# arcee-ai/DALM

Hardware: NVIDIA H100
Metric: RAG-e2e train-step samples/sec (bge-large + Llama-2-7B, bs=18) (higher is better)
Workload: dtype bf16

## Files before the change

### dalm_b200/csrc/gemm_wgmma.cu

```cuda
#include "common.cuh"
#include "ptx.cuh"
#include <cudaTypedefs.h>
#include <mutex>
#include <unordered_map>

namespace dalm {
using namespace ptx;

enum class Epi {
  Plain,
  SwiGLU,
  RoPE,
  GeluPair,
  NormRoPE,
};

struct GemmEpilogue {
  void* out;
  long long ldo;
  int out_f32;
  const float* bias;
  const void* resid;
  long long ldr;
  int resid_f32;
  int act;
  float alpha;
  int M, N, K;
  DropCfg drop;
  int group_m;
  const float* rope_cos; const float* rope_sin;
  int rope_L, rope_cols;
  const float* q_norm; const float* k_norm;
  int nq_heads;
  float norm_eps;
  float* norm_rstd; long long ld_rstd;
  int norm_pre;
  int l2_hints;
};

__device__ __forceinline__ void tile_coords(int tile, int num_m, int num_n, int gm, int& m_blk, int& n_blk) {
  if (gm <= 0) { m_blk = tile % num_m; n_blk = tile / num_m; return; }
  const int band_tiles = gm * num_n;
  const int band = tile / band_tiles;
  const int r = tile - band * band_tiles;
  const int m0 = band * gm;
  const int h = min(gm, num_m - m0);
  const int n = r / h;
  m_blk = m0 + (r - n * h);
  n_blk = (band & 1) ? (num_n - 1 - n) : n;
}

template <bool PRE = false>
__device__ __forceinline__ void epilogue_math(const GemmEpilogue& ep, const uint32_t* v, float* f, int row, int col0, bool row_ok,
                                              const float4* rpre = nullptr) {
  const int N = ep.N;
#pragma unroll
  for (int i = 0; i < 32; ++i) f[i] = __uint_as_float(v[i]) * ep.alpha;
  if (ep.bias) {
#pragma unroll
    for (int i = 0; i < 32; ++i) if (col0 + i < N) f[i] += __ldg(ep.bias + col0 + i);
  }
  if (ep.act == 1) {
#pragma unroll
    for (int i = 0; i < 32; ++i) f[i] = gelu_erf(f[i]);
  }
  if (ep.drop.p > 0.f) {
    const unsigned long long dstream = drop_stream(ep.drop);
    const unsigned long long base = ((unsigned long long)row * (unsigned long long)N + (unsigned long long)col0) >> 3;
#pragma unroll
    for (int g = 0; g < 4; ++g) {
      float sc[8];
      drop_scale8(ep.drop, dstream, base + g, sc);
#pragma unroll
      for (int j = 0; j < 8; ++j) f[g * 8 + j] *= sc[j];
    }
  }
  if constexpr (PRE) {
#pragma unroll
    for (int g = 0; g < 8; ++g) { f[g * 4 + 0] += rpre[g].x; f[g * 4 + 1] += rpre[g].y; f[g * 4 + 2] += rpre[g].z; f[g * 4 + 3] += rpre[g].w; }
  } else if (ep.resid && row_ok) {
    if (ep.resid_f32) {
      const float* r = reinterpret_cast<const float*>(ep.resid) + (size_t)row * ep.ldr + col0;
#pragma unroll
      for (int g = 0; g < 8; ++g) {
        if (col0 + g * 4 < N) {
          const float4 t = *reinterpret_cast<const float4*>(r + g * 4);
          f[g * 4 + 0] += t.x; f[g * 4 + 1] += t.y; f[g * 4 + 2] += t.z; f[g * 4 + 3] += t.w;
        }
      }
    } else {
      const __nv_bfloat16* r = reinterpret_cast<const __nv_bfloat16*>(ep.resid) + (size_t)row * ep.ldr + col0;
#pragma unroll
      for (int g = 0; g < 4; ++g) {
        if (col0 + g * 8 < N) {
          const bf16x8 t = *reinterpret_cast<const bf16x8*>(r + g * 8);
          float tf[8];
          unpack8(t, tf);
          if (ep.act == 2) {
#pragma unroll
            for (int i = 0; i < 8; ++i) f[g * 8 + i] = __bfloat162float(__float2bfloat16_rn(f[g * 8 + i])) * gelu_erf_grad(tf[i]);
          } else {
#pragma unroll
            for (int i = 0; i < 8; ++i) f[g * 8 + i] += tf[i];
          }
        }
      }
    }
  }
}

__device__ __forceinline__ void acc_ld32(const float* p, uint32_t* v) {
#pragma unroll
  for (int g = 0; g < 8; ++g) {
    const float4 t = *reinterpret_cast<const float4*>(p + g * 4);
    v[g * 4 + 0] = __float_as_uint(t.x); v[g * 4 + 1] = __float_as_uint(t.y);
    v[g * 4 + 2] = __float_as_uint(t.z); v[g * 4 + 3] = __float_as_uint(t.w);
  }
}

constexpr int kStageTileBytes = 128 * 128;
constexpr int kEpiGroups = 2;
constexpr int kGemmThreads = 128 + kEpiGroups * 128;
template <int BN, Epi EPI>
__device__ __forceinline__ void epilogue_drain_tile(const GemmEpilogue& ep, const CUtensorMap* tmap_out, const CUtensorMap* tmap_out2,
                                                    unsigned char* staging, int grp, const float* arow, int row_in_tile, int tile_row0,
                                                    int tile_col0) {
  static_assert(BN == 256 || EPI == Epi::Plain || EPI == Epi::GeluPair, "the SwiGLU and RoPE epilogues need 256-wide tiles");
  const int N = ep.N;
  const int row = tile_row0 + row_in_tile;
  const bool row_ok = row < ep.M;
  constexpr bool F32_OUT = EPI == Epi::Plain;
  const int sb_cols = (F32_OUT && ep.out_f32) ? 32 : 64;
  const bool issuer = (threadIdx.x == 128 + grp * 128);
  unsigned char* tile = staging + grp * kStageTileBytes;
  unsigned char* st = tile + row_in_tile * 128;
  const int sw = row_in_tile & 7;
  const bool rpf = F32_OUT && ep.out_f32 && ep.resid != nullptr && ep.resid_f32;
  float4 rnext[8];
  auto fetch_resid = [&](int cc) {
    const int cg0 = tile_col0 + cc;
    const float* r = reinterpret_cast<const float*>(ep.resid) + (size_t)row * ep.ldr + cg0;
#pragma unroll
    for (int g = 0; g < 8; ++g)
      rnext[g] = (row_ok && cc < BN && cg0 + g * 4 < N) ? *reinterpret_cast<const float4*>(r + g * 4) : make_float4(0.f, 0.f, 0.f, 0.f);
  };
  if (rpf) fetch_resid(grp * sb_cols);
#pragma unroll 1
  for (int c = grp * sb_cols; c < BN; c += kEpiGroups * sb_cols) {
    const int col0 = tile_col0 + c;
    if (col0 >= N) break;
    if (issuer) bulk_wait_read<0>();
    named_bar_sync(1 + grp, 128);
    if (F32_OUT && ep.out_f32) {
      uint32_t v[32]; float f[32];
      acc_ld32(arow + c, v);
      if (rpf) {
        epilogue_math<true>(ep, v, f, row, col0, row_ok, rnext);
        fetch_resid(c + kEpiGroups * sb_cols);
      } else {
        epilogue_math<false>(ep, v, f, row, col0, row_ok);
      }
#pragma unroll
      for (int g = 0; g < 8; ++g)
        *reinterpret_cast<float4*>(st + ((g ^ sw) << 4)) = make_float4(f[g * 4], f[g * 4 + 1], f[g * 4 + 2], f[g * 4 + 3]);
    } else if (EPI == Epi::RoPE && col0 < ep.rope_cols) {
      const bool second = ((col0 >> 6) & 1) != 0;
      const int cp = second ? c - 64 : c + 64;
      const int colp = tile_col0 + cp;
      const int pos = row_ok ? (row % ep.rope_L) : 0;
      const float* cs = ep.rope_cos + (size_t)pos * 64;
      const float* sn = ep.rope_sin + (size_t)pos * 64;
#pragma unroll
      for (int h = 0; h < 2; ++h) {
        uint32_t vo[32], vq[32]; float f[32];
        acc_ld32(arow + (c + h * 32), vo);
        acc_ld32(arow + (cp + h * 32), vq);
        float cc[32], ss[32];
#pragma unroll
        for (int i = 0; i < 32; i += 4) {
          *reinterpret_cast<float4*>(cc + i) = __ldg(reinterpret_cast<const float4*>(cs + h * 32 + i));
          *reinterpret_cast<float4*>(ss + i) = __ldg(reinterpret_cast<const float4*>(sn + h * 32 + i));
        }
#pragma unroll
        for (int i = 0; i < 32; ++i) {
          float own = __uint_as_float(vo[i]), oth = __uint_as_float(vq[i]);
          if (ep.bias) {
            own += __ldg(ep.bias + col0 + h * 32 + i);
            oth += __ldg(ep.bias + colp + h * 32 + i);
          }
          f[i] = second ? fmaf(own, cc[i], oth * ss[i]) : fmaf(own, cc[i], -oth * ss[i]);
        }
#pragma unroll
        for (int g = 0; g < 4; ++g)
          *reinterpret_cast<bf16x8*>(st + (((h * 4 + g) ^ sw) << 4)) = pack8(f + g * 8);
      }
    } else if (EPI == Epi::NormRoPE && col0 < ep.rope_cols) {
      const bool second = ((col0 >> 6) & 1) != 0;
      const int cp = second ? c - 64 : c + 64;
      const int colp = tile_col0 + cp;
      const int c1 = second ? cp : c;
      const int head = col0 >> 7;
      const float* nw = head < ep.nq_heads ? ep.q_norm : ep.k_norm;
      const int jo = second ? 64 : 0, jp = 64 - jo;
      float ss = 0.f;
#pragma unroll 1
      for (int h = 0; h < 4; ++h) {
        uint32_t v[32];
        acc_ld32(arow + (c1 + h * 32), v);
#pragma unroll
        for (int i = 0; i < 32; ++i) {
          float x = __uint_as_float(v[i]);
          if (ep.bias) x += __ldg(ep.bias + tile_col0 + c1 + h * 32 + i);
          ss = fmaf(x, x, ss);
        }
      }
      const float rstd = rsqrtf(ss * (1.f / 128.f) + ep.norm_eps);
      if (ep.norm_rstd && row_ok && !second) ep.norm_rstd[(size_t)row * ep.ld_rstd + head] = rstd;
      const int pos = row_ok ? (row % ep.rope_L) : 0;
      const float* cs = ep.rope_cos + (size_t)pos * 64;
      const float* sn = ep.rope_sin + (size_t)pos * 64;
#pragma unroll
      for (int h = 0; h < 2; ++h) {
        uint32_t vo[32], vq[32]; float f[32];
        acc_ld32(arow + (c + h * 32), vo);
        acc_ld32(arow + (cp + h * 32), vq);
        float cc[32], ss2[32];
#pragma unroll
        for (int i = 0; i < 32; i += 4) {
          *reinterpret_cast<float4*>(cc + i) = __ldg(reinterpret_cast<const float4*>(cs + h * 32 + i));
          *reinterpret_cast<float4*>(ss2 + i) = __ldg(reinterpret_cast<const float4*>(sn + h * 32 + i));
        }
#pragma unroll
        for (int i = 0; i < 32; ++i) {
          float own = __uint_as_float(vo[i]), oth = __uint_as_float(vq[i]);
          if (ep.bias) {
            own += __ldg(ep.bias + col0 + h * 32 + i);
            oth += __ldg(ep.bias + colp + h * 32 + i);
          }
          own = own * rstd * __ldg(nw + jo + h * 32 + i);
          oth = oth * rstd * __ldg(nw + jp + h * 32 + i);
          f[i] = second ? fmaf(own, cc[i], oth * ss2[i]) : fmaf(own, cc[i], -oth * ss2[i]);
        }
#pragma unroll
        for (int g = 0; g < 4; ++g)
          *reinterpret_cast<bf16x8*>(st + (((h * 4 + g) ^ sw) << 4)) = pack8(f + g * 8);
      }
      fence_proxy_async();
      named_bar_sync(1 + grp, 128);
      if (issuer) {
        if (ep.l2_hints & 4) tma_store_2d_hint(tmap_out, tile, col0, tile_row0, l2_policy_evict_first());
        else                 tma_store_2d(tmap_out, tile, col0, tile_row0);
        bulk_commit();
      }
      if (!ep.norm_pre) continue;
      if (issuer) bulk_wait_read<0>();
      named_bar_sync(1 + grp, 128);
#pragma unroll
      for (int h = 0; h < 2; ++h) {
        uint32_t v[32]; float f[32];
        acc_ld32(arow + (c + h * 32), v);
#pragma unroll
        for (int i = 0; i < 32; ++i) {
          f[i] = __uint_as_float(v[i]);
          if (ep.bias) f[i] += __ldg(ep.bias + col0 + h * 32 + i);
        }
#pragma unroll
        for (int g = 0; g < 4; ++g)
          *reinterpret_cast<bf16x8*>(st + (((h * 4 + g) ^ sw) << 4)) = pack8(f + g * 8);
      }
      fence_proxy_async();
      named_bar_sync(1 + grp, 128);
      if (issuer) {
        tma_store_2d(tmap_out2, tile, col0, tile_row0);
        bulk_commit();
      }
      continue;
    } else if (EPI == Epi::GeluPair) {
      bf16x8 pk[8];
#pragma unroll
      for (int h = 0; h < 2; ++h) {
        if (col0 + h * 32 < N) {
          uint32_t v[32]; float f[32];
          acc_ld32(arow + (c + h * 32), v);
          epilogue_math(ep, v, f, row, col0 + h * 32, row_ok);
#pragma unroll
          for (int g = 0; g < 4; ++g) pk[h * 4 + g] = pack8(f + g * 8);
        } else {
#pragma unroll
          for (int g = 0; g < 4; ++g) pk[h * 4 + g] = bf16x8{};
        }
      }
#pragma unroll
      for (int g = 0; g < 8; ++g) *reinterpret_cast<bf16x8*>(st + ((g ^ sw) << 4)) = pk[g];
      fence_proxy_async();
      named_bar_sync(1 + grp, 128);
      if (issuer) {
        if (ep.l2_hints & 4) tma_store_2d_hint(tmap_out, tile, col0, tile_row0, l2_policy_evict_first());
        else                 tma_store_2d(tmap_out, tile, col0, tile_row0);
        bulk_commit();
      }
#pragma unroll
      for (int g = 0; g < 8; ++g) {
        float x[8];
        unpack8(pk[g], x);
#pragma unroll
        for (int i = 0; i < 8; ++i) x[i] = gelu_erf(x[i]);
        pk[g] = pack8(x);
      }
      if (issuer) bulk_wait_read<0>();
      named_bar_sync(1 + grp, 128);
#pragma unroll
      for (int g = 0; g < 8; ++g) *reinterpret_cast<bf16x8*>(st + ((g ^ sw) << 4)) = pk[g];
      fence_proxy_async();
      named_bar_sync(1 + grp, 128);
      if (issuer) {
        tma_store_2d(tmap_out2, tile, col0, tile_row0);
        bulk_commit();
      }
      continue;
    } else {
#pragma unroll
      for (int h = 0; h < 2; ++h) {
        if (col0 + h * 32 < N) {
          uint32_t v[32]; float f[32];
          acc_ld32(arow + (c + h * 32), v);
          epilogue_math(ep, v, f, row, col0 + h * 32, row_ok);
#pragma unroll
          for (int g = 0; g < 4; ++g)
            *reinterpret_cast<bf16x8*>(st + (((h * 4 + g) ^ sw) << 4)) = pack8(f + g * 8);
        }
      }
    }
    fence_proxy_async();
    named_bar_sync(1 + grp, 128);
    if (issuer) {
      if (ep.l2_hints & 4) tma_store_2d_hint(tmap_out, tile, col0, tile_row0, l2_policy_evict_first());
      else                 tma_store_2d(tmap_out, tile, col0, tile_row0);
      bulk_commit();
    }
  }
  if constexpr (EPI == Epi::SwiGLU) {
    const int j = grp;
    const int acol0 = (tile_col0 >> 1) + j * 64;
    if (issuer) bulk_wait_read<0>();
    named_bar_sync(1 + grp, 128);
#pragma unroll
    for (int h = 0; h < 2; ++h) {
      uint32_t vg[32], vu[32]; float f[32];
      acc_ld32(arow + (j * 64 + h * 32), vg);
      acc_ld32(arow + (128 + j * 64 + h * 32), vu);
#pragma unroll
      for (int i = 0; i < 32; ++i) {
        const float g = __uint_as_float(vg[i]);
        f[i] = g / (1.f + __expf(-g)) * __uint_as_float(vu[i]);
      }
#pragma unroll
      for (int g4 = 0; g4 < 4; ++g4) *reinterpret_cast<bf16x8*>(st + (((h * 4 + g4) ^ sw) << 4)) = pack8(f + g4 * 8);
    }
    fence_proxy_async();
    named_bar_sync(1 + grp, 128);
    if (issuer) {
      if (ep.l2_hints & 4) tma_store_2d_hint(tmap_out2, tile, acol0, tile_row0, l2_policy_evict_first());
      else                 tma_store_2d(tmap_out2, tile, acol0, tile_row0);
      bulk_commit();
    }
  }
}

template <int BN> struct GemmCfg {
  static constexpr int BM = 128, BK = 64;
  static constexpr int A_BYTES = BM * BK * 2;
  static constexpr int B_BYTES = BN * BK * 2;
  static constexpr int STAGE_BYTES = A_BYTES + B_BYTES;
  static constexpr int STAGES = (BN == 256) ? 4 : (BN == 128 ? 6 : 8);
  static constexpr int ACC_LD = BN + 4;
  static constexpr int SMEM_BYTES = STAGES * STAGE_BYTES + 2 * kStageTileBytes + 1024  + 256 ;
  static_assert(BM * ACC_LD * 4 <= STAGES * STAGE_BYTES, "the accumulator tile reuses the stage ring");
  static_assert(SMEM_BYTES <= 232448, "exceeds 227 KB of shared memory per block");
};

template <int BN, int TA, int TB>
__device__ __forceinline__ void wgmma_tile(float* d, uint64_t da, uint64_t db, int scale_d) {
  if constexpr (BN == 256) wgmma_m64n256k16<TA, TB>(d, da, db, scale_d);
  else if constexpr (BN == 128) wgmma_m64n128k16<TA, TB>(d, da, db, scale_d);
  else wgmma_m64n64k16<TA, TB>(d, da, db, scale_d);
}

template <int BN, int LAYOUT, Epi EPI, int CL>
__global__ void __launch_bounds__(kGemmThreads, 1)
gemm_bf16_tn_kernel(const __grid_constant__ CUtensorMap tmap_a, const __grid_constant__ CUtensorMap tmap_b,
                    const __grid_constant__ CUtensorMap tmap_out, const __grid_constant__ CUtensorMap tmap_out2, const GemmEpilogue ep) {
  using Cfg = GemmCfg<BN>;
  constexpr int BM = Cfg::BM, BK = Cfg::BK, STAGES = Cfg::STAGES;
  static_assert(CL == 1 || (LAYOUT == 0 && EPI == Epi::Plain), "the cluster kernel takes the plain TN layout");
  extern __shared__ unsigned char smem_raw[];
  unsigned char* smem = reinterpret_cast<unsigned char*>((reinterpret_cast<uintptr_t>(smem_raw) + 1023) & ~uintptr_t(1023));
  unsigned char* staging = smem + STAGES * Cfg::STAGE_BYTES;
  uint64_t* full_bar  = reinterpret_cast<uint64_t*>(staging + 2 * kStageTileBytes);
  uint64_t* empty_bar = full_bar + STAGES;
  uint64_t* epi_bar   = empty_bar + STAGES;
  float* acc_smem = reinterpret_cast<float*>(smem);

  const int warp = threadIdx.x >> 5, lane = threadIdx.x & 31;
  const uint32_t rank = CL == 2 ? cluster_ctarank() : 0u;
  const int M = ep.M, N = ep.N, K = ep.K;
  const int num_m = (M + CL * BM - 1) / (CL * BM), num_n = (N + BN - 1) / BN;
  const int num_tiles = num_m * num_n;
  const int num_kb = (K + BK - 1) / BK;
  const int unit = blockIdx.x / CL, num_units = gridDim.x / CL;
  const int group_m = CL == 2 ? 0 : ep.group_m;

  if (threadIdx.x == 0) {
    prefetch_tmap(&tmap_a);
    prefetch_tmap(&tmap_b);
    prefetch_tmap(&tmap_out);
    if constexpr (EPI == Epi::SwiGLU || EPI == Epi::GeluPair || EPI == Epi::NormRoPE) prefetch_tmap(&tmap_out2);
  }
  if (threadIdx.x == 32) {
    for (int s = 0; s < STAGES; ++s) { mbar_init(&full_bar[s], 1); mbar_init(&empty_bar[s], 8 * CL); }
    mbar_init(epi_bar, 8 * CL);
    fence_mbar_init();
  }
  if constexpr (CL == 2) cluster_sync_all();
  else __syncthreads();

  if (warp < 4) {
    asm volatile("setmaxnreg.dec.sync.aligned.u32 40;" ::: "memory");
    if (warp == 0 && lane == 0) {
      int stage = 0; uint32_t phase = 0;
      const bool hint_a = (ep.l2_hints & 1) != 0, hint_b = (ep.l2_hints & 2) != 0;
      const uint64_t pol_a = hint_a ? l2_policy_evict_last() : 0ull, pol_b = hint_b ? l2_policy_evict_first() : 0ull;
      auto load = [](void* dst, const CUtensorMap* tm, uint64_t* bar, int c0, int c1, bool hinted, uint64_t pol) {
        if (hinted) tma_load_2d_hint(dst, tm, bar, c0, c1, pol);
        else        tma_load_2d(dst, tm, bar, c0, c1);
      };
      int it = 0;
      for (int tile = unit; tile < num_tiles; tile += num_units, ++it) {
        int m_blk, n_blk;
        tile_coords(tile, num_m, num_n, group_m, m_blk, n_blk);
        if (it > 0) mbar_wait(epi_bar, (uint32_t)(it - 1) & 1u);
        for (int kb = 0; kb < num_kb; ++kb) {
          mbar_wait(&empty_bar[stage], phase ^ 1);
          unsigned char* sa = smem + stage * Cfg::STAGE_BYTES;
          unsigned char* sb = sa + Cfg::A_BYTES;
          mbar_arrive_expect_tx(&full_bar[stage], Cfg::STAGE_BYTES);
          if constexpr (CL == 2) {
            load(sa, &tmap_a, &full_bar[stage], kb * BK, (m_blk * CL + (int)rank) * BM, hint_a, pol_a);
            tma_load_2d_multicast(sb + rank * (Cfg::B_BYTES / 2), &tmap_b, &full_bar[stage], kb * BK, n_blk * BN + (int)rank * (BN / 2), 0x3);
          } else {
            if constexpr (LAYOUT == 2) {
#pragma unroll
              for (int c = 0; c < BM / 64; ++c) load(sa + c * 8192, &tmap_a, &full_bar[stage], m_blk * BM + c * 64, kb * BK, hint_a, pol_a);
            } else {
              load(sa, &tmap_a, &full_bar[stage], kb * BK, m_blk * BM, hint_a, pol_a);
            }
            if constexpr (LAYOUT >= 1) {
#pragma unroll
              for (int c = 0; c < BN / 64; ++c) load(sb + c * 8192, &tmap_b, &full_bar[stage], n_blk * BN + c * 64, kb * BK, hint_b, pol_b);
            } else {
              load(sb, &tmap_b, &full_bar[stage], kb * BK, n_blk * BN, hint_b, pol_b);
            }
          }
          if (++stage == STAGES) { stage = 0; phase ^= 1; }
        }
      }
    }
  } else {
    asm volatile("setmaxnreg.inc.sync.aligned.u32 232;" ::: "memory");
    const int grp = (warp - 4) >> 2;
    const int q = warp & 3;
    constexpr int TA = LAYOUT == 2 ? 1 : 0, TB = LAYOUT >= 1 ? 1 : 0;
    constexpr uint64_t a_step = TA ? 128 : 2, b_step = TB ? 128 : 2;
    const uint32_t a_off = (uint32_t)grp * 8192u;
    int stage = 0; uint32_t phase = 0;
    for (int tile = unit; tile < num_tiles; tile += num_units) {
      int m_blk, n_blk;
      tile_coords(tile, num_m, num_n, group_m, m_blk, n_blk);
      float acc[BN / 2];
      int prev = -1;
      for (int kb = 0; kb < num_kb; ++kb) {
        mbar_wait(&full_bar[stage], phase);
        const uint32_t sa = smem_u32(smem + stage * Cfg::STAGE_BYTES);
        const uint32_t sb = sa + Cfg::A_BYTES;
        const uint64_t adesc = TA ? make_sw128_mnmajor_desc(sa + a_off, 8192, 1024) : make_sw128_kmajor_desc(sa + a_off);
        const uint64_t bdesc = TB ? make_sw128_mnmajor_desc(sb, 8192, 1024) : make_sw128_kmajor_desc(sb);
        wgmma_fence();
#pragma unroll
        for (int k = 0; k < BK / 16; ++k)
          wgmma_tile<BN, TA, TB>(acc, adesc + a_step * (uint64_t)k, bdesc + b_step * (uint64_t)k, (kb | k) != 0 ? 1 : 0);
        wgmma_commit();
        wgmma_wait<1>();
        if (prev >= 0 && lane == 0) {
          mbar_arrive(&empty_bar[prev]);
          if constexpr (CL == 2) mbar_arrive_remote(&empty_bar[prev], rank ^ 1u);
        }
        prev = stage;
        if (++stage == STAGES) { stage = 0; phase ^= 1; }
      }
      wgmma_wait<0>();
      if (lane == 0) {
        mbar_arrive(&empty_bar[prev]);
        if constexpr (CL == 2) mbar_arrive_remote(&empty_bar[prev], rank ^ 1u);
      }
      named_bar_sync(3, 256);
      {
        const int r0 = grp * 64 + q * 16 + (lane >> 2);
        float* p0 = acc_smem + (size_t)r0 * Cfg::ACC_LD + 2 * (lane & 3);
        float* p1 = p0 + 8 * Cfg::ACC_LD;
#pragma unroll
        for (int j = 0; j < BN / 8; ++j) {
          *reinterpret_cast<float2*>(p0 + 8 * j) = make_float2(acc[4 * j], acc[4 * j + 1]);
          *reinterpret_cast<float2*>(p1 + 8 * j) = make_float2(acc[4 * j + 2], acc[4 * j + 3]);
        }
      }
      named_bar_sync(3, 256);
      const int row_in_tile = q * 32 + lane;
      epilogue_drain_tile<BN, EPI>(ep, &tmap_out, &tmap_out2, staging, grp, acc_smem + (size_t)row_in_tile * Cfg::ACC_LD,
                                   row_in_tile, (m_blk * CL + (int)rank) * BM, n_blk * BN);
      fence_proxy_async();
      __syncwarp();
      if (lane == 0) {
        mbar_arrive(epi_bar);
        if constexpr (CL == 2) mbar_arrive_remote(epi_bar, rank ^ 1u);
      }
    }
    if ((threadIdx.x & 127) == 0) bulk_wait<0>();
  }
  if constexpr (CL == 2) cluster_sync_all();
}

static PFN_cuTensorMapEncodeTiled_v12000 get_encode_fn() {
  static PFN_cuTensorMapEncodeTiled_v12000 fn = nullptr;
  static std::once_flag once;
  std::call_once(once, [] {
    void* p = nullptr;
    cudaDriverEntryPointQueryResult qres;
    if (cudaGetDriverEntryPoint("cuTensorMapEncodeTiled", &p, cudaEnableDefault, &qres) == cudaSuccess &&
        qres == cudaDriverEntryPointSuccess)
      fn = reinterpret_cast<PFN_cuTensorMapEncodeTiled_v12000>(p);
  });
  return fn;
}

struct TmapKey {
  const void* ptr; long long rows, cols, ld; int box_rows; int f32;
  bool operator==(const TmapKey& o) const {
    return ptr == o.ptr && rows == o.rows && cols == o.cols && ld == o.ld && box_rows == o.box_rows && f32 == o.f32;
  }
};
struct TmapKeyHash {
  size_t operator()(const TmapKey& k) const {
    size_t h = reinterpret_cast<size_t>(k.ptr);
    h = h * 1000003u ^ (size_t)k.rows; h = h * 1000003u ^ (size_t)k.cols;
    h = h * 1000003u ^ (size_t)k.ld;   h = h * 1000003u ^ (size_t)(k.box_rows * 2 + k.f32);
    return h;
  }
};
static std::unordered_map<TmapKey, CUtensorMap, TmapKeyHash> g_tmaps;
static std::mutex g_tmap_mu;

int get_tmap(const void* ptr, long long rows, long long cols, long long ld, int box_rows, CUtensorMap* out, int f32) {
  TmapKey key{ptr, rows, cols, ld, box_rows, f32};
  {
    std::lock_guard<std::mutex> g(g_tmap_mu);
    auto it = g_tmaps.find(key);
    if (it != g_tmaps.end()) { *out = it->second; return 0; }
  }
  auto fn = get_encode_fn();
  DALM_REQUIRE(fn != nullptr, "gemm: cuTensorMapEncodeTiled driver entry point unavailable");
  DALM_REQUIRE((reinterpret_cast<uintptr_t>(ptr) & 15) == 0, "gemm: operand base %p is not 16-byte aligned", ptr);
  DALM_REQUIRE((ld % (f32 ? 4 : 8)) == 0, "gemm: row stride %lld is not a multiple of 16 bytes", ld);
  cuuint64_t dims[2] = {(cuuint64_t)cols, (cuuint64_t)rows};
  cuuint64_t strides[1] = {(cuuint64_t)ld * (f32 ? 4 : 2)};
  cuuint32_t box[2] = {f32 ? 32u : 64u, (cuuint32_t)box_rows};
  cuuint32_t estr[2] = {1u, 1u};
  CUtensorMap m;
  CUresult r = fn(&m, f32 ? CU_TENSOR_MAP_DATA_TYPE_FLOAT32 : CU_TENSOR_MAP_DATA_TYPE_BFLOAT16, 2, const_cast<void*>(ptr), dims, strides, box, estr,
                  CU_TENSOR_MAP_INTERLEAVE_NONE, CU_TENSOR_MAP_SWIZZLE_128B, CU_TENSOR_MAP_L2_PROMOTION_L2_256B,
                  CU_TENSOR_MAP_FLOAT_OOB_FILL_NONE);
  DALM_REQUIRE(r == CUDA_SUCCESS, "gemm: cuTensorMapEncodeTiled failed (%d) rows=%lld cols=%lld ld=%lld box_rows=%d",
               (int)r, rows, cols, ld, box_rows);
  {
    std::lock_guard<std::mutex> g(g_tmap_mu);
    if (g_tmaps.size() > 8192) g_tmaps.clear();
    g_tmaps[key] = m;
  }
  *out = m;
  return 0;
}

template <int BN, int LAYOUT, Epi EPI>
static int launch_gemm(const CUtensorMap& ta, const CUtensorMap& tb, const CUtensorMap& to, const GemmEpilogue& ep,
                       int max_ctas, cudaStream_t stream, const CUtensorMap* to2) {
  using Cfg = GemmCfg<BN>;
  static bool attr_set = false;
  if (!attr_set) {
    DALM_CUDA(cudaFuncSetAttribute(gemm_bf16_tn_kernel<BN, LAYOUT, EPI, 1>, cudaFuncAttributeMaxDynamicSharedMemorySize, Cfg::SMEM_BYTES));
    attr_set = true;
  }
  const int num_tiles = ((ep.M + 127) / 128) * ((ep.N + BN - 1) / BN);
  int grid = num_tiles < num_sms() ? num_tiles : num_sms();
  if (max_ctas > 0 && grid > max_ctas) grid = max_ctas;
  gemm_bf16_tn_kernel<BN, LAYOUT, EPI, 1><<<grid, kGemmThreads, Cfg::SMEM_BYTES, stream>>>(ta, tb, to, to2 ? *to2 : to, ep);
  count_launch();
  return check_launch("gemm_bf16_tn_kernel");
}

template <int LAYOUT, Epi EPI>
static int launch_gemm_bn(int bn, const CUtensorMap& ta, const CUtensorMap& tb, const CUtensorMap& to, const GemmEpilogue& ep,
                          int max_ctas, cudaStream_t stream, const CUtensorMap* to2 = nullptr) {
  if (bn == 256) return launch_gemm<256, LAYOUT, EPI>(ta, tb, to, ep, max_ctas, stream, to2);
  if (bn == 128) return launch_gemm<128, LAYOUT, EPI>(ta, tb, to, ep, max_ctas, stream, to2);
  return launch_gemm<64, LAYOUT, EPI>(ta, tb, to, ep, max_ctas, stream, to2);
}

template <int BN>
static int launch_gemm_cluster(const CUtensorMap& ta, const CUtensorMap& tb, const CUtensorMap& to, const GemmEpilogue& ep,
                               int max_ctas, cudaStream_t stream) {
  using Cfg = GemmCfg<BN>;
  auto kern = gemm_bf16_tn_kernel<BN, 0, Epi::Plain, 2>;
  static bool attr_set = false;
  if (!attr_set) {
    DALM_CUDA(cudaFuncSetAttribute(kern, cudaFuncAttributeMaxDynamicSharedMemorySize, Cfg::SMEM_BYTES));
    attr_set = true;
  }
  const int num_tiles = ((ep.M + 255) / 256) * ((ep.N + BN - 1) / BN);
  int clusters = num_tiles < num_sms() / 2 ? num_tiles : num_sms() / 2;
  if (max_ctas > 0 && clusters > max_ctas / 2) clusters = max_ctas / 2 > 0 ? max_ctas / 2 : 1;
  cudaLaunchConfig_t cfg = {};
  cfg.gridDim = dim3(2 * clusters);
  cfg.blockDim = dim3(kGemmThreads);
  cfg.dynamicSmemBytes = Cfg::SMEM_BYTES;
  cfg.stream = stream;
  cudaLaunchAttribute attr[1];
  attr[0].id = cudaLaunchAttributeClusterDimension;
  attr[0].val.clusterDim.x = 2; attr[0].val.clusterDim.y = 1; attr[0].val.clusterDim.z = 1;
  cfg.attrs = attr; cfg.numAttrs = 1;
  DALM_CUDA(cudaLaunchKernelEx(&cfg, kern, ta, tb, to, to, ep));
  count_launch();
  return check_launch("gemm_bf16_tn_kernel (cluster of 2)");
}

}

using namespace dalm;

static int env_int(const char* name, int dflt) {
  const char* v = getenv(name);
  return (v && *v) ? atoi(v) : dflt;
}
static int g_group_m_override = env_int("DALM_B200_GEMM_RASTER", 0);
extern "C" void dalm_b200_gemm_set_raster(int group_m) { g_group_m_override = group_m; }
static int g_l2_hints = env_int("DALM_B200_GEMM_L2_HINTS", -1);
static double l2_resident_a() { return (double)l2_bytes() / 3.0; }
extern "C" void dalm_b200_gemm_set_l2_hints(int mask) { g_l2_hints = mask < 0 ? -1 : (mask & 7); }
static int pick_l2_hints(int M, int N, int K, int tile_n, int group_m, bool stream_out) {
  if (g_l2_hints >= 0) return g_l2_hints;
  const long long tiles = (long long)((M + 127) / 128) * ((N + tile_n - 1) / tile_n);
  return (group_m == 0 && tiles > num_sms() && 2.0 * M * K <= l2_resident_a() && !stream_out) ? 7 : 0;
}

static int pick_block_n(int M, int N) {
  const long long m1 = (M + 127) / 128;
  double best = 1e30;
  int bn = 64;
  const int cand[3] = {256, 128, 64};
  const double penalty[3] = {1.0, 1.55, 2.7};
  for (int i = 0; i < 3; ++i) {
    if (cand[i] > 64 && N < cand[i]) continue;
    const long long tiles = m1 * ((N + cand[i] - 1) / cand[i]);
    const double cost = (double)((tiles + num_sms() - 1) / num_sms()) * cand[i] * penalty[i];
    if (cost < best) { best = cost; bn = cand[i]; }
  }
  return bn;
}

static int pick_group_m(int M, int N, int K, int tile_n, bool stream_out) {
  const int num_m = (M + 127) / 128, num_n = (N + tile_n - 1) / tile_n;
  int group_m = 0;
  if (g_group_m_override > 0) return g_group_m_override;
  if (g_group_m_override == -1 || (long long)num_m * num_n <= num_sms()) return 0;
  const double a_bytes = 2.0 * M * K;
  if (g_group_m_override == 0 && a_bytes <= l2_resident_a() && !stream_out) return 0;
  const double ideal = sqrt((double)num_sms() * tile_n / 128.0);
  int nbands = (int)(num_m / ideal + 0.5);
  if (nbands < 1) nbands = 1;
  group_m = (num_m + nbands - 1) / nbands;
  if (group_m >= num_m) group_m = 0;
  return group_m;
}

static GemmEpilogue gemm_epilogue(int M, int N, int K, int tile_n, void* out, long long ldo, int out_f32 = 0,
                                  const void* resid = nullptr, long long ldr = 0, int resid_f32 = 0) {
  GemmEpilogue ep{};
  ep.out = out; ep.ldo = ldo; ep.out_f32 = out_f32;
  ep.resid = resid; ep.ldr = ldr; ep.resid_f32 = resid_f32;
  ep.alpha = 1.f;
  ep.M = M; ep.N = N; ep.K = K;
  ep.drop = make_drop(0.f, 0, 0, nullptr);
  const bool stream_out = out_f32 != 0 || resid != nullptr;
  ep.group_m = pick_group_m(M, N, K, tile_n, stream_out);
  ep.l2_hints = pick_l2_hints(M, N, K, tile_n, ep.group_m, stream_out);
  return ep;
}

extern "C" int dalm_b200_gemm_bf16(int layout, const void* A, long long lda, const void* B, long long ldb, void* out,
                                   long long ldo, int out_f32, int M, int N, int K, float alpha, const float* bias,
                                   int act, const void* resid, long long ldr, int resid_f32, int block_n,
                                   int max_ctas, float drop_p, unsigned long long drop_seed,
                                   unsigned long long drop_stream_id, const void* drop_offset, void* stream) {
  DALM_REQUIRE(layout >= 0 && layout <= 2, "gemm: layout must be 0 (TN), 1 (NN) or 2 (wgrad)");
  DALM_REQUIRE(M > 0 && N > 0 && K > 0, "gemm: empty problem M=%d N=%d K=%d", M, N, K);
  DALM_REQUIRE((N % 8) == 0, "gemm: N=%d must be a multiple of 8", N);
  DALM_REQUIRE((K % 8) == 0 || layout == 2, "gemm: K=%d must be a multiple of 8", K);
  DALM_REQUIRE((M % 8) == 0 || layout != 2, "gemm: M=%d must be a multiple of 8 for the wgrad layout", M);
  DALM_REQUIRE(lda >= (layout == 2 ? M : K) && ldb >= (layout >= 1 ? N : K) && ldo >= N, "gemm: leading dimensions too small");
  DALM_REQUIRE((ldo % (out_f32 ? 4 : 8)) == 0, "gemm: ldo=%lld breaks 16-byte row alignment", ldo);
  DALM_REQUIRE((reinterpret_cast<uintptr_t>(out) & 15) == 0, "gemm: out is not 16-byte aligned");
  if (resid) {
    DALM_REQUIRE((ldr % (resid_f32 ? 4 : 8)) == 0, "gemm: ldr=%lld breaks 16-byte row alignment", ldr);
    DALM_REQUIRE((reinterpret_cast<uintptr_t>(resid) & 15) == 0, "gemm: resid is not 16-byte aligned");
  }
  DALM_REQUIRE(act == 0 || act == 1 || act == 2, "gemm: act must be 0 (none), 1 (gelu) or 2 (gelu backward: multiply by gelu'(resid))");
  DALM_REQUIRE(act != 2 || (resid != nullptr && !resid_f32 && !out_f32 && drop_p == 0.f),
               "gemm: act 2 (gelu backward) needs a bf16 `resid` (the pre-activation), a bf16 output and no dropout");
  int bn = block_n;
  if (bn == 0) bn = pick_block_n(M, N);
  DALM_REQUIRE(bn == 64 || bn == 128 || bn == 256 || bn == 2128 || bn == 2256,
               "gemm: block_n must be 0, 64/128/256 (single CTA) or 2128/2256 (cluster of two CTAs)");
  const bool pair = bn > 1000;
  DALM_REQUIRE(!(pair && layout != 0), "gemm: the cluster kernel only takes the TN layout");
  const int tile_n = pair ? bn % 1000 : bn;
  CUtensorMap ta, tb, to;
  if (layout == 2) { if (int e = get_tmap(A, K, M, lda, 64, &ta)) return e; }
  else             { if (int e = get_tmap(A, M, K, lda, 128, &ta)) return e; }
  if (layout >= 1) { if (int e = get_tmap(B, K, N, ldb, 64, &tb)) return e; }
  else             { if (int e = get_tmap(B, N, K, ldb, pair ? tile_n / 2 : tile_n, &tb)) return e; }
  if (int e = get_tmap(out, M, N, ldo, 128, &to, out_f32)) return e;
  DALM_REQUIRE(drop_p >= 0.f && drop_p < 1.f, "gemm: dropout p must be in [0,1)");
  GemmEpilogue ep = gemm_epilogue(M, N, K, tile_n, out, ldo, out_f32, resid, ldr, resid_f32);
  ep.bias = bias; ep.act = act; ep.alpha = alpha;
  ep.drop = make_drop(drop_p, drop_seed, drop_stream_id, drop_offset);
  cudaStream_t st = (cudaStream_t)stream;
  if (bn == 2256) return launch_gemm_cluster<256>(ta, tb, to, ep, max_ctas, st);
  if (bn == 2128) return launch_gemm_cluster<128>(ta, tb, to, ep, max_ctas, st);
  if (layout == 1) return launch_gemm_bn<1, Epi::Plain>(bn, ta, tb, to, ep, max_ctas, st);
  if (layout == 2) return launch_gemm_bn<2, Epi::Plain>(bn, ta, tb, to, ep, max_ctas, st);
  return launch_gemm_bn<0, Epi::Plain>(bn, ta, tb, to, ep, max_ctas, st);
}

extern "C" int dalm_b200_gemm_bf16_swiglu(const void* A, long long lda, const void* B, long long ldb, void* gu, long long ldgu,
                                          void* act, long long ldact, int M, int N, int K, void* stream) {
  DALM_REQUIRE(M > 0 && K > 0 && N >= 256 && (N % 256) == 0, "gemm_swiglu: N=%d must be a positive multiple of 256 (128-feature gate / up blocks)", N);
  DALM_REQUIRE((K % 8) == 0 && lda >= K && ldb >= K && ldgu >= N && ldact >= N / 2, "gemm_swiglu: bad K / leading dimensions");
  DALM_REQUIRE((ldgu % 8) == 0 && (ldact % 8) == 0 && ((uintptr_t)gu & 15) == 0 && ((uintptr_t)act & 15) == 0, "gemm_swiglu: output alignment");
  CUtensorMap ta, tb, to, to2;
  if (int e = get_tmap(A, M, K, lda, 128, &ta)) return e;
  if (int e = get_tmap(B, N, K, ldb, 256, &tb)) return e;
  if (int e = get_tmap(gu, M, N, ldgu, 128, &to, 0)) return e;
  if (int e = get_tmap(act, M, N / 2, ldact, 128, &to2, 0)) return e;
  const GemmEpilogue ep = gemm_epilogue(M, N, K, 256, gu, ldgu);
  return launch_gemm<256, 0, Epi::SwiGLU>(ta, tb, to, ep, 0, (cudaStream_t)stream, &to2);
}

extern "C" int dalm_b200_gemm_bf16_gelu(const void* A, long long lda, const void* B, long long ldb, void* pre, long long ldpre,
                                        void* act, long long ldact, int M, int N, int K, const float* bias, void* stream) {
  DALM_REQUIRE(M > 0 && N > 0 && K > 0 && (N % 8) == 0 && (K % 8) == 0, "gemm_gelu: bad shape M=%d N=%d K=%d", M, N, K);
  DALM_REQUIRE(lda >= K && ldb >= K && ldpre >= N && ldact >= N, "gemm_gelu: leading dimensions too small");
  DALM_REQUIRE((ldpre % 8) == 0 && (ldact % 8) == 0 && ((uintptr_t)pre & 15) == 0 && ((uintptr_t)act & 15) == 0, "gemm_gelu: output alignment");
  const int bn = pick_block_n(M, N);
  CUtensorMap ta, tb, to, to2;
  if (int e = get_tmap(A, M, K, lda, 128, &ta)) return e;
  if (int e = get_tmap(B, N, K, ldb, bn, &tb)) return e;
  if (int e = get_tmap(pre, M, N, ldpre, 128, &to, 0)) return e;
  if (int e = get_tmap(act, M, N, ldact, 128, &to2, 0)) return e;
  GemmEpilogue ep = gemm_epilogue(M, N, K, bn, pre, ldpre);
  ep.bias = bias;
  return launch_gemm_bn<0, Epi::GeluPair>(bn, ta, tb, to, ep, 0, (cudaStream_t)stream, &to2);
}

extern "C" int dalm_b200_gemm_bf16_rope(const void* A, long long lda, const void* B, long long ldb, void* out, long long ldo, int M,
                                        int N, int K, const float* bias, const float* cos_t, const float* sin_t, int L, int rope_cols,
                                        const float* q_norm, const float* k_norm, int nq_heads, float eps, void* pre_out,
                                        long long ld_pre, float* rstd_out, long long ld_rstd, void* stream) {
  DALM_REQUIRE(M > 0 && N > 0 && K > 0 && (N % 8) == 0 && (K % 8) == 0, "gemm_rope: bad shape M=%d N=%d K=%d", M, N, K);
  DALM_REQUIRE(rope_cols > 0 && rope_cols <= N && (rope_cols % 256) == 0, "gemm_rope: rope_cols=%d must be a multiple of 256 (whole 128-wide heads per tile)", rope_cols);
  DALM_REQUIRE(L > 0 && cos_t != nullptr && sin_t != nullptr && ((uintptr_t)cos_t & 15) == 0 && ((uintptr_t)sin_t & 15) == 0, "gemm_rope: cos / sin tables");
  DALM_REQUIRE(lda >= K && ldb >= K && ldo >= N && (ldo % 8) == 0 && ((uintptr_t)out & 15) == 0, "gemm_rope: leading dimensions / alignment");
  CUtensorMap ta, tb, to;
  if (int e = get_tmap(A, M, K, lda, 128, &ta)) return e;
  if (int e = get_tmap(B, N, K, ldb, 256, &tb)) return e;
  if (int e = get_tmap(out, M, N, ldo, 128, &to, 0)) return e;
  GemmEpilogue ep = gemm_epilogue(M, N, K, 256, out, ldo);
  ep.bias = bias;
  ep.rope_cos = cos_t; ep.rope_sin = sin_t; ep.rope_L = L; ep.rope_cols = rope_cols;
  if (q_norm == nullptr) {
    DALM_REQUIRE(k_norm == nullptr && pre_out == nullptr && rstd_out == nullptr, "gemm_rope: k_norm / pre_out / rstd_out need q_norm");
    return launch_gemm<256, 0, Epi::RoPE>(ta, tb, to, ep, 0, (cudaStream_t)stream, nullptr);
  }
  DALM_REQUIRE(k_norm != nullptr && nq_heads >= 0 && nq_heads <= rope_cols / 128 && eps >= 0.f, "gemm_rope: norm weights / nq_heads=%d", nq_heads);
  DALM_REQUIRE(rstd_out == nullptr || ld_rstd >= rope_cols / 128, "gemm_rope: ld_rstd=%lld < %d heads", ld_rstd, rope_cols / 128);
  CUtensorMap to2 = to;
  if (pre_out != nullptr) {
    DALM_REQUIRE(ld_pre >= rope_cols && (ld_pre % 8) == 0 && ((uintptr_t)pre_out & 15) == 0, "gemm_rope: pre_out leading dimension / alignment");
    if (int e = get_tmap(pre_out, M, rope_cols, ld_pre, 128, &to2, 0)) return e;
  }
  ep.q_norm = q_norm; ep.k_norm = k_norm; ep.nq_heads = nq_heads; ep.norm_eps = eps;
  ep.norm_rstd = rstd_out; ep.ld_rstd = ld_rstd; ep.norm_pre = pre_out != nullptr;
  return launch_gemm<256, 0, Epi::NormRoPE>(ta, tb, to, ep, 0, (cudaStream_t)stream, &to2);
}

extern "C" void dalm_b200_gemm_clear_cache() {
  std::lock_guard<std::mutex> g(g_tmap_mu);
  g_tmaps.clear();
}
```

Baseline: 72.21.

## Drain RoPE GEMM epilogue directly from registers, skipping accumulator parking in shared memory

Result: faster. 72.97 (median of 6 runs) (+1.0%).

```diff
diff --git a/dalm_b200/csrc/gemm_wgmma.cu b/dalm_b200/csrc/gemm_wgmma.cu
--- a/dalm_b200/csrc/gemm_wgmma.cu
+++ b/dalm_b200/csrc/gemm_wgmma.cu
@@ -125,7 +125,8 @@
 __device__ __forceinline__ void epilogue_drain_tile(const GemmEpilogue& ep, const CUtensorMap* tmap_out, const CUtensorMap* tmap_out2,
                                                     unsigned char* staging, int grp, const float* arow, int row_in_tile, int tile_row0,
                                                     int tile_col0) {
-  static_assert(BN == 256 || EPI == Epi::Plain || EPI == Epi::GeluPair, "the SwiGLU and RoPE epilogues need 256-wide tiles");
+  static_assert(BN == 256 || EPI == Epi::Plain || EPI == Epi::GeluPair, "the SwiGLU and NormRoPE epilogues need 256-wide tiles");
+  static_assert(EPI != Epi::RoPE, "Epi::RoPE drains from registers (epilogue_registers_rope)");
   const int N = ep.N;
   const int row = tile_row0 + row_in_tile;
   const bool row_ok = row < ep.M;
@@ -163,37 +164,6 @@
 #pragma unroll
       for (int g = 0; g < 8; ++g)
         *reinterpret_cast<float4*>(st + ((g ^ sw) << 4)) = make_float4(f[g * 4], f[g * 4 + 1], f[g * 4 + 2], f[g * 4 + 3]);
-    } else if (EPI == Epi::RoPE && col0 < ep.rope_cols) {
-      const bool second = ((col0 >> 6) & 1) != 0;
-      const int cp = second ? c - 64 : c + 64;
-      const int colp = tile_col0 + cp;
-      const int pos = row_ok ? (row % ep.rope_L) : 0;
-      const float* cs = ep.rope_cos + (size_t)pos * 64;
-      const float* sn = ep.rope_sin + (size_t)pos * 64;
-#pragma unroll
-      for (int h = 0; h < 2; ++h) {
-        uint32_t vo[32], vq[32]; float f[32];
-        acc_ld32(arow + (c + h * 32), vo);
-        acc_ld32(arow + (cp + h * 32), vq);
-        float cc[32], ss[32];
-#pragma unroll
-        for (int i = 0; i < 32; i += 4) {
-          *reinterpret_cast<float4*>(cc + i) = __ldg(reinterpret_cast<const float4*>(cs + h * 32 + i));
-          *reinterpret_cast<float4*>(ss + i) = __ldg(reinterpret_cast<const float4*>(sn + h * 32 + i));
-        }
-#pragma unroll
-        for (int i = 0; i < 32; ++i) {
-          float own = __uint_as_float(vo[i]), oth = __uint_as_float(vq[i]);
-          if (ep.bias) {
-            own += __ldg(ep.bias + col0 + h * 32 + i);
-            oth += __ldg(ep.bias + colp + h * 32 + i);
-          }
-          f[i] = second ? fmaf(own, cc[i], oth * ss[i]) : fmaf(own, cc[i], -oth * ss[i]);
-        }
-#pragma unroll
-        for (int g = 0; g < 4; ++g)
-          *reinterpret_cast<bf16x8*>(st + (((h * 4 + g) ^ sw) << 4)) = pack8(f + g * 8);
-      }
     } else if (EPI == Epi::NormRoPE && col0 < ep.rope_cols) {
       const bool second = ((col0 >> 6) & 1) != 0;
       const int cp = second ? c - 64 : c + 64;
@@ -364,6 +334,108 @@
       else                 tma_store_2d(tmap_out2, tile, acol0, tile_row0);
       bulk_commit();
     }
+  }
+}
+
+constexpr int kStageBufBytes = 64 * 128;
+constexpr int kRegBoxRows = 64;
+
+__device__ __forceinline__ int swz128(int r, int b) { return r * 128 + (((b >> 4) ^ (r & 7)) << 4) + (b & 15); }
+
+struct EpiStager {
+  unsigned char* base;
+  uint32_t n;
+  bool issuer;
+  uint32_t bar;
+  __device__ __forceinline__ unsigned char* acquire() {
+    if (issuer) bulk_wait_read<1>();
+    named_bar_sync(bar, 128);
+    return base + (n & 1) * kStageBufBytes;
+  }
+  __device__ __forceinline__ void store(const CUtensorMap* tm, int c0, int r0, bool evict_first) {
+    fence_proxy_async();
+    named_bar_sync(bar, 128);
+    if (issuer) {
+      const unsigned char* src = base + (n & 1) * kStageBufBytes;
+      if (evict_first) tma_store_2d_hint(tm, src, c0, r0, l2_policy_evict_first());
+      else             tma_store_2d(tm, src, c0, r0);
+      bulk_commit();
+    }
+    ++n;
+  }
+};
+
+__device__ __forceinline__ void stage_bf16(unsigned char* buf, const float* v, int rl, int cq) {
+#pragma unroll
+  for (int i = 0; i < 16; ++i)
+    *reinterpret_cast<__nv_bfloat162*>(buf + swz128(rl + 8 * (i & 1), 2 * (8 * (i >> 1) + cq))) = __floats2bfloat162_rn(v[2 * i], v[2 * i + 1]);
+}
+
+template <int S>
+__device__ __forceinline__ void acc_shift(float* acc) {
+#pragma unroll
+  for (int i = 0; i + S < 128; ++i) acc[i] = acc[i + S];
+}
+
+__device__ __forceinline__ void epilogue_registers_rope(const GemmEpilogue& ep, float* acc, const CUtensorMap* tmap_out,
+                                                        EpiStager& sg, int row0, int tile_col0) {
+  const int N = ep.N;
+  const int lane = threadIdx.x & 31;
+  const int rl = 16 * ((threadIdx.x >> 5) & 3) + (lane >> 2);
+  const int cq = 2 * (lane & 3);
+  const bool evict = (ep.l2_hints & 4) != 0;
+  if (tile_col0 < ep.rope_cols) {
+    const float* cs[2]; const float* sn[2];
+#pragma unroll
+    for (int h = 0; h < 2; ++h) {
+      const int row = row0 + rl + 8 * h;
+      const int pos = row < ep.M ? row % ep.rope_L : 0;
+      cs[h] = ep.rope_cos + (size_t)pos * 64 + cq;
+      sn[h] = ep.rope_sin + (size_t)pos * 64 + cq;
+    }
+#pragma unroll 1
+    for (int hd = 0; hd < 2; ++hd) {
+#pragma unroll 1
+      for (int half = 0; half < 2; ++half) {
+        const int col0 = tile_col0 + 128 * hd + 64 * half;
+        float v[32];
+#pragma unroll
+        for (int i = 0; i < 16; ++i) {
+          const int jj = i >> 1, h = i & 1, col = col0 + 8 * jj + cq, colp = col ^ 64;
+          float x0 = half ? acc[32 + 4 * jj + 2 * h] : acc[4 * jj + 2 * h];
+          float x1 = half ? acc[32 + 4 * jj + 2 * h + 1] : acc[4 * jj + 2 * h + 1];
+          float y0 = half ? acc[4 * jj + 2 * h] : acc[32 + 4 * jj + 2 * h];
+          float y1 = half ? acc[4 * jj + 2 * h + 1] : acc[32 + 4 * jj + 2 * h + 1];
+          if (ep.bias) {
+            x0 += __ldg(ep.bias + col); x1 += __ldg(ep.bias + col + 1);
+            y0 += __ldg(ep.bias + colp); y1 += __ldg(ep.bias + colp + 1);
+          }
+          const float2 c = __ldg(reinterpret_cast<const float2*>(cs[h] + 8 * jj));
+          const float2 s = __ldg(reinterpret_cast<const float2*>(sn[h] + 8 * jj));
+          if (half) { x0 = fmaf(x0, c.x, y0 * s.x);  x1 = fmaf(x1, c.y, y1 * s.y); }
+          else      { x0 = fmaf(x0, c.x, -y0 * s.x); x1 = fmaf(x1, c.y, -y1 * s.y); }
+          v[2 * i] = x0; v[2 * i + 1] = x1;
+        }
+        stage_bf16(sg.acquire(), v, rl, cq);
+        sg.store(tmap_out, col0, row0, evict);
+      }
+      acc_shift<64>(acc);
+    }
+    return;
+  }
+#pragma unroll 1
+  for (int col0 = tile_col0; col0 < tile_col0 + 256 && col0 < N; col0 += 64) {
+    float v[32];
+#pragma unroll
+    for (int i = 0; i < 16; ++i) {
+      const int jj = i >> 1, h = i & 1, col = col0 + 8 * jj + cq;
+      float x0 = acc[4 * jj + 2 * h], x1 = acc[4 * jj + 2 * h + 1];
+      if (ep.bias && col < N) { x0 += __ldg(ep.bias + col); x1 += __ldg(ep.bias + col + 1); }
+      v[2 * i] = x0; v[2 * i + 1] = x1;
+    }
+    stage_bf16(sg.acquire(), v, rl, cq);
+    sg.store(tmap_out, col0, row0, evict);
+    acc_shift<32>(acc);
   }
 }
 
@@ -400,6 +472,7 @@
   uint64_t* empty_bar = full_bar + STAGES;
   uint64_t* epi_bar   = empty_bar + STAGES;
   float* acc_smem = reinterpret_cast<float*>(smem);
+  constexpr bool PARK = EPI != Epi::RoPE;
 
   const int warp = threadIdx.x >> 5, lane = threadIdx.x & 31;
   const uint32_t rank = CL == 2 ? cluster_ctarank() : 0u;
@@ -438,7 +511,7 @@
       for (int tile = unit; tile < num_tiles; tile += num_units, ++it) {
         int m_blk, n_blk;
         tile_coords(tile, num_m, num_n, group_m, m_blk, n_blk);
-        if (it > 0) mbar_wait(epi_bar, (uint32_t)(it - 1) & 1u);
+        if (PARK && it > 0) mbar_wait(epi_bar, (uint32_t)(it - 1) & 1u);
         for (int kb = 0; kb < num_kb; ++kb) {
           mbar_wait(&empty_bar[stage], phase ^ 1);
           unsigned char* sa = smem + stage * Cfg::STAGE_BYTES;
@@ -473,6 +546,7 @@
     constexpr uint64_t a_step = TA ? 128 : 2, b_step = TB ? 128 : 2;
     const uint32_t a_off = (uint32_t)grp * 8192u;
     int stage = 0; uint32_t phase = 0;
+    EpiStager sg{staging + grp * kStageTileBytes, 0u, (threadIdx.x & 127) == 0, 1u + (uint32_t)grp};
     for (int tile = unit; tile < num_tiles; tile += num_units) {
       int m_blk, n_blk;
       tile_coords(tile, num_m, num_n, group_m, m_blk, n_blk);
@@ -502,26 +576,30 @@
         mbar_arrive(&empty_bar[prev]);
         if constexpr (CL == 2) mbar_arrive_remote(&empty_bar[prev], rank ^ 1u);
       }
-      named_bar_sync(3, 256);
-      {
-        const int r0 = grp * 64 + q * 16 + (lane >> 2);
-        float* p0 = acc_smem + (size_t)r0 * Cfg::ACC_LD + 2 * (lane & 3);
-        float* p1 = p0 + 8 * Cfg::ACC_LD;
-#pragma unroll
-        for (int j = 0; j < BN / 8; ++j) {
-          *reinterpret_cast<float2*>(p0 + 8 * j) = make_float2(acc[4 * j], acc[4 * j + 1]);
-          *reinterpret_cast<float2*>(p1 + 8 * j) = make_float2(acc[4 * j + 2], acc[4 * j + 3]);
-        }
-      }
-      named_bar_sync(3, 256);
-      const int row_in_tile = q * 32 + lane;
-      epilogue_drain_tile<BN, EPI>(ep, &tmap_out, &tmap_out2, staging, grp, acc_smem + (size_t)row_in_tile * Cfg::ACC_LD,
-                                   row_in_tile, (m_blk * CL + (int)rank) * BM, n_blk * BN);
-      fence_proxy_async();
-      __syncwarp();
-      if (lane == 0) {
-        mbar_arrive(epi_bar);
-        if constexpr (CL == 2) mbar_arrive_remote(epi_bar, rank ^ 1u);
+      if constexpr (!PARK) {
+        epilogue_registers_rope(ep, acc, &tmap_out, sg, (m_blk * CL + (int)rank) * BM + 64 * grp, n_blk * BN);
+      } else {
+        named_bar_sync(3, 256);
+        {
+          const int r0 = grp * 64 + q * 16 + (lane >> 2);
+          float* p0 = acc_smem + (size_t)r0 * Cfg::ACC_LD + 2 * (lane & 3);
+          float* p1 = p0 + 8 * Cfg::ACC_LD;
+#pragma unroll
+          for (int j = 0; j < BN / 8; ++j) {
+            *reinterpret_cast<float2*>(p0 + 8 * j) = make_float2(acc[4 * j], acc[4 * j + 1]);
+            *reinterpret_cast<float2*>(p1 + 8 * j) = make_float2(acc[4 * j + 2], acc[4 * j + 3]);
+          }
+        }
+        named_bar_sync(3, 256);
+        const int row_in_tile = q * 32 + lane;
+        epilogue_drain_tile<BN, EPI>(ep, &tmap_out, &tmap_out2, staging, grp, acc_smem + (size_t)row_in_tile * Cfg::ACC_LD,
+                                     row_in_tile, (m_blk * CL + (int)rank) * BM, n_blk * BN);
+        fence_proxy_async();
+        __syncwarp();
+        if (lane == 0) {
+          mbar_arrive(epi_bar);
+          if constexpr (CL == 2) mbar_arrive_remote(epi_bar, rank ^ 1u);
+        }
       }
     }
     if ((threadIdx.x & 127) == 0) bulk_wait<0>();
@@ -790,7 +868,7 @@
   CUtensorMap ta, tb, to;
   if (int e = get_tmap(A, M, K, lda, 128, &ta)) return e;
   if (int e = get_tmap(B, N, K, ldb, 256, &tb)) return e;
-  if (int e = get_tmap(out, M, N, ldo, 128, &to, 0)) return e;
+  if (int e = get_tmap(out, M, N, ldo, q_norm ? 128 : kRegBoxRows, &to, 0)) return e;
   GemmEpilogue ep = gemm_epilogue(M, N, K, 256, out, ldo);
   ep.bias = bias;
   ep.rope_cos = cos_t; ep.rope_sin = sin_t; ep.rope_L = L; ep.rope_cols = rope_cols;
```
